# menezesandre/stackrl

Measured on AMD Instinct MI355X. Metric: env steps/sec (batched Stack-v0), higher is better.
Workload: dtype f32

## Files before the change

stackrl_amd/csrc/settle.hip:

```cpp
#include "srl_device.h"
#include "srl_kernels.h"
#include "stage.h"

#ifdef SRL_DIAG_JITTER
__device__ __forceinline__ void srl_jitter_sync() {
  unsigned t = (unsigned)__builtin_readcyclecounter() * 2654435761u + (threadIdx.x >> 6) * 40503u;
  t = __builtin_amdgcn_readfirstlane(t);
  const int n = (t >> 13) & 15;
  for (int i = 0; i < n; ++i) __builtin_amdgcn_s_sleep(16);
  __builtin_amdgcn_fence(__ATOMIC_RELEASE, "workgroup");
  __builtin_amdgcn_s_barrier();
  __builtin_amdgcn_fence(__ATOMIC_ACQUIRE, "workgroup");
  t = t * 1664525u + 1013904223u;
  const int m = (t >> 13) & 15;
  for (int i = 0; i < m; ++i) __builtin_amdgcn_s_sleep(16);
}
#define __syncthreads() srl_jitter_sync()
#endif

template <int T, int PP> struct Variant;

__device__ __forceinline__ int pair_word(int p) {
  int j = (int)((1.0f + sqrtf(1.0f + 8.0f * (float)p)) * 0.5f);
  while (j * (j - 1) / 2 > p) --j;
// ... 424 lines not shown
      if (flags & 2) {
        for (int pid = 0; pid < npair; ++pid) {
          if (L.SOP()[pid] >= 0) continue;
          int i, j; L.pair(pid, i, j);
          if (!aabb_overlap(L, i, j)) continue;
          int sl = -1;
          for (int k = 0; k < P.NS; ++k) if (L.POS()[k] < 0) { sl = k; break; }
          if (sl < 0) { misc[M_STATUS] |= SRL_ST_PAIR_OVERFLOW; atomicOr(P.flags, 4); continue; }
          L.SOP()[pid] = sl; L.POS()[sl] = pid;
          float* mp = L.MAN(sl);
          mp[0] = __int_as_float(0);
          mp[56] = __int_as_float(0);
          st3(mp + 1, ld3(L.X(i)) - ld3(L.X(j)));
        }
      }
      uint64_t* used = (uint64_t*)(L.sm + P.BLOB + P.S_USED);
      for (int b = 0; b < SRL_MAX_BODIES; ++b) used[b] = 0;
      int nc = 0;
      for (int sl = 0; sl < P.NS; ++sl) {
        int pid = L.POS()[sl];
        if (pid < 0) continue;
        int i, j; L.pair(pid, i, j);
        uint64_t u = used[i] | used[j];
        int c = __ffsll((long long)~u) - 1;
        L.COL()[sl] = c;
        used[i] |= (uint64_t)1 << c;
        used[j] |= (uint64_t)1 << c;
        if (c + 1 > nc) nc = c + 1;
      }
      misc[M_NCOL] = nc;
    }
    __syncthreads();
  }
  const int ncol = misc[M_NCOL];
  STAMP(3);
  {
    constexpr int G = VA::GJK_GROUP;
    const int gl = tid & (G - 1);
    for (int sl = tid / G; sl < P.NS; sl += T / G)
      if (L.POS()[sl] >= 0) narrowphase_slot<G>(L, sl, gl);
  }
  __syncthreads();
  STAMP(4);
  {
    GPoint gp = make_ground_point(L, tid / SRL_GMAXP, tid % SRL_GMAXP);
    if (tid / SRL_GMAXP >= nb) gp.valid = false;
    Point pp[PP];
    PSplit sp;
    if constexpr (VA::PAIR_SPLIT) {
#pragma unroll
      for (int r = 0; r < PP; ++r) pp[r].valid = slot_points(L, tid >> 2) > 0;
    } else {
#pragma unroll
    for (int r = 0; r < PP; ++r) pp[r] = make_pair_point(L, (tid + r * T) >> 2, tid & 3);
    }
    {
      bool mine = gp.valid;
#pragma unroll
      for (int r = 0; r < PP; ++r) mine |= pp[r].valid;
      if (tid >= 64 && __ballot(mine) != 0ull && (tid & 63) == 0) misc[M_SOLO] = 0;
    }
    __syncthreads();
    GBody gb;
    gb.np = 0; gb.b = 0; gb.ima = 0.0f;
    gb.pvw = L.VW(0); gb.rec = cg_rec(L, 0, 0);
#pragma unroll
    for (int i = 0; i < SRL_GMAXP; ++i) { gb.acc[i][0] = 0.0f; gb.acc[i][1] = 0.0f; gb.acc[i][2] = 0.0f; }
    constexpr bool GB = VA::GROUND_BODY, GA = VA::GROUND_AHEAD;
    if (GB) {
    if (gp.valid) cg_store(L, gp);
    if (tid < nb) {
      const float* g = L.GM(tid);
      gb.b = tid; gb.np = __float_as_int(g[0]); gb.ima = L.BC(tid)[0];
      gb.pvw = L.VW(tid); gb.rec = cg_rec(L, tid, 0);
#pragma unroll
      for (int i = 0; i < SRL_GMAXP; ++i)
        if (i < gb.np) { gb.acc[i][0] = g[SRL_GM_IN + i]; gb.acc[i][1] = g[SRL_GM_T1 + i]; gb.acc[i][2] = g[SRL_GM_T2 + i]; }
    }
    __syncthreads();
    }
    if constexpr (VA::PAIR_SPLIT) sp = make_pair_split(L, tid);
    STAMP(5);
    const bool solo = VA::SOLO && misc[M_SOLO] != 0;
    const int gslot = gp.valid ? gp.idx : -1;
    unsigned long long cm[2], cm2[2] = {0ull, 0ull};
    int pslot[PP];
    if constexpr (VA::PAIR_SPLIT) {
      const int h2 = (tid >> 1) & 1;
#pragma unroll
      for (int c = 0; c < 2; ++c) {
        cm[c] = __ballot(sp.colour == c && sp.np > 2 * h2); cm2[c] = __ballot(sp.colour == c && sp.np > 2 * h2 + 1);
      }
#pragma unroll
      for (int r = 0; r < PP; ++r) pslot[r] = -1;
    } else {
    cm[0] = __ballot(pp[0].valid && pp[0].colour == 0); cm[1] = __ballot(pp[0].valid && pp[0].colour == 1);
#pragma unroll
    for (int r = 0; r < PP; ++r) pslot[r] = pp[r].valid ? 4 * pp[r].colour + pp[r].idx : -1;
    }
    if (solo) {
      int done = 0;
      if (tid < 64) {
        bool anyp = false;
#pragma unroll
        for (int r = 0; r < PP; ++r) anyp |= pp[r].valid;
        const bool ground_only = GB && __ballot(anyp) == 0ull;
        if (ground_only) {
          v3 v = V(0.0f, 0.0f, 0.0f), w = V(0.0f, 0.0f, 0.0f);
          if (gb.np > 0) {
            vw_load(gb.pvw, v, w);
            float res = 0.0f;
            ground_body<true, false, true>(gb, P.c.warmstart, v, w, res);
          }
          for (int it = 0; it < P.c.solver_iterations; ++it) {
            done++;
            float res = 0.0f;
            if (gb.np > 0) ground_body<false, GA, true>(gb, P.c.warmstart, v, w, res);
            if (__ballot(res * res > P.c.residual_threshold) == 0ull) break;
          }
          if (gb.np > 0) vw_store(gb.pvw, v, w);
        } else {
          solver_sweep<true, T, PP, VA::SOLO>(L, gp, gb, pp, sp, ncol, gslot, pslot, 0, cm, cm2);
          for (int it = 0; it < P.c.solver_iterations; ++it) {
            done++;
            if (!solver_sweep<false, T, PP, VA::SOLO>(L, gp, gb, pp, sp, ncol, gslot, pslot, 0, cm, cm2)) break;
          }
        }
        if (tid == 0) misc[M_CNT] = done;
      }
      __syncthreads();
      gsweep += misc[M_CNT];
    } else {
      solver_sweep<true, T, PP, false>(L, gp, gb, pp, sp, ncol, gslot, pslot, 0, cm, cm2);
      for (int it = 0; it < P.c.solver_iterations; ++it) {
        gsweep++;
        if (!solver_sweep<false, T, PP, false>(L, gp, gb, pp, sp, ncol, gslot, pslot, gsweep, cm, cm2)) break;
      }
    }
#ifdef SRL_STAMPS
    if (tid == 0) {
      EnvHdr* hh = &L.P->hdr[blockIdx.x];
      bool anyp = false;
      for (int r = 0; r < PP; ++r) anyp |= pp[r].valid;
      {
        int bl[SRL_MAX_BODIES]; for (int b = 0; b < SRL_MAX_BODIES; ++b) bl[b] = 0;
        int lmax = 0, sumt = 0;
        for (int c = 0; c < ncol; ++c) {
          int mx = 0;
          for (int sl = 0; sl < P.NS; ++sl) {
            const int pid = L.POS()[sl];
            if (pid < 0 || L.COL()[sl] != c) continue;
            const int np = __float_as_int(L.MAN(sl)[0]);
            if (np <= 0) continue;
            int a, b; L.pair(pid, a, b);
            const int st = bl[a] > bl[b] ? bl[a] : bl[b];
            bl[a] = st + np; bl[b] = st + np;
            if (st + np > lmax) lmax = st + np;
            if (np > mx) mx = np;
          }
          sumt += mx;
        }
        hh->diag[4] += sumt; hh->diag[5] += lmax;
      }
      hh->diag[0] += 1; hh->diag[1] += (__ballot(anyp) == 0ull); hh->diag[2] += ncol; hh->diag[3] += solo ? misc[M_CNT] : 0;
    }
#endif
    if (!GB) {
      if (gp.valid) { float* g = L.GM(gp.a); g[SRL_GM_IN + gp.idx] = gp.in; g[SRL_GM_T1 + gp.idx] = gp.i1; g[SRL_GM_T2 + gp.idx] = gp.i2; }
    } else if (gb.np > 0) {
      float* g = L.GM(gb.b);
#pragma unroll
      for (int i = 0; i < SRL_GMAXP; ++i)
        if (i < gb.np) { g[SRL_GM_IN + i] = gb.acc[i][0]; g[SRL_GM_T1 + i] = gb.acc[i][1]; g[SRL_GM_T2 + i] = gb.acc[i][2]; }
    }
    if constexpr (VA::PAIR_SPLIT) {
      const int i0 = tid & 2;
      if (!(tid & 1) && sp.np > i0) {
        float* q = L.MAN(tid >> 2) + 4 + SRL_MP_WORDS * i0;
        q[10] = sp.s0.in; q[11] = sp.s0.i1; q[12] = sp.s0.i2;
        if (sp.np > i0 + 1) { q[SRL_MP_WORDS + 10] = sp.s1.in; q[SRL_MP_WORDS + 11] = sp.s1.i1; q[SRL_MP_WORDS + 12] = sp.s1.i2; }
      }
    } else {
#pragma unroll
    for (int r = 0; r < PP; ++r)
      if (pp[r].valid) {
        float* q = L.MAN((tid + r * T) >> 2) + 4 + SRL_MP_WORDS * pp[r].idx;
        q[10] = pp[r].in; q[11] = pp[r].i1; q[12] = pp[r].i2;
      }
    }
  }
  STAMP(6);
  const float dt = P.c.sim_time_step;
  if (tid < nb) {
    const int b = tid;
    v3 v, w;
    vw_load(L.VW(b), v, w);
    st3(L.X(b), madd(ld3(L.X(b)), v, dt));
    float* Q = L.Q(b);
    q4 q; q.x = Q[0]; q.y = Q[1]; q.z = Q[2]; q.w = Q[3];
    float hx = 0.5f * dt;
    q4 dq;
    dq.x = hx * ((w.x * q.w + w.y * q.z) - w.z * q.y);
    dq.y = hx * ((w.y * q.w + w.z * q.x) - w.x * q.z);
    dq.z = hx * ((w.z * q.w + w.x * q.y) - w.y * q.x);
    dq.w = hx * (-((w.x * q.x + w.y * q.y) + w.z * q.z));
    q.x += dq.x; q.y += dq.y; q.z += dq.z; q.w += dq.w;
    float inv = 1.0f / sqrtf((q.x * q.x + q.y * q.y) + (q.z * q.z + q.w * q.w));
    Q[0] = q.x * inv; Q[1] = q.y * inv; Q[2] = q.z * inv; Q[3] = q.w * inv;
  }
  __syncthreads();
  STAMP(7);
}

__device__ __forceinline__ bool sim_stop(const Lds& L, int nb, int tid) {
  int* misc = L.MISC();
  bool moving = false;
  if (tid < nb) {
    const float* p = L.VW(tid); const v3 v = V(p[0], p[2], p[4]);
    moving = sqrtf(dot(v, v)) > L.P->c.velocity_threshold;
// ... 376 lines not shown
```

stackrl_amd/csrc/solver.h:

```cpp
struct Row { v3 d, ca, aa, cb, ab; float rk, k; };

template <bool HAS_B>
__device__ __forceinline__ Row make_row(v3 d, v3 ra, v3 rb, float ima, const m3& Ia, float imb, const m3& Ib) {
  Row r;
  r.d = d;
  r.ca = cross(ra, d);
  r.aa = mmul(Ia, r.ca);
  r.cb = V(0.0f, 0.0f, 0.0f); r.ab = V(0.0f, 0.0f, 0.0f);
  float k = ima + dot(cross(r.aa, ra), d);
  if (HAS_B) {
    r.cb = cross(rb, d);
    r.ab = mmul(Ib, r.cb);
    k = k + (imb + dot(cross(r.ab, rb), d));
  }
  r.rk = 1.0f / k;
  r.k = k;
  return r;
}

struct PRow { f2 ka[3], kb[3], ua[3], ub[3]; float rk, k; };
struct Vel2 { f2 a[3], b[3]; };

__device__ __forceinline__ PRow pack_row(const Row& r, float ima, float imb) {
  PRow q;
  const v3 da = r.d * ima, db = r.d * (-imb);
  q.ka[0] = F2(r.d.x, r.ca.x); q.ka[1] = F2(r.d.y, r.ca.y); q.ka[2] = F2(r.d.z, r.ca.z);
  q.kb[0] = F2(r.d.x, r.cb.x); q.kb[1] = F2(r.d.y, r.cb.y); q.kb[2] = F2(r.d.z, r.cb.z);
  q.ua[0] = F2(da.x, r.aa.x); q.ua[1] = F2(da.y, r.aa.y); q.ua[2] = F2(da.z, r.aa.z);
  q.ub[0] = F2(db.x, -r.ab.x); q.ub[1] = F2(db.y, -r.ab.y); q.ub[2] = F2(db.z, -r.ab.z);
  q.rk = r.rk; q.k = r.k;
  return q;
}

__device__ __forceinline__ void prow_apply(const PRow& r, Vel2& u, float imp) {
  const f2 d2 = F2(imp, imp);
#pragma unroll
  for (int c = 0; c < 3; ++c) { u.a[c] = fma2(r.ua[c], d2, u.a[c]); u.b[c] = fma2(r.ub[c], d2, u.b[c]); }
}
__device__ __forceinline__ void prow_solve(const PRow& r, Vel2& u, float target, float& acc, float lo, float hi, float& res) {
  const f2 sa = fma2(r.ka[0], u.a[0], fma2(r.ka[1], u.a[1], r.ka[2] * u.a[2]));
  const f2 sb = fma2(r.kb[0], u.b[0], fma2(r.kb[1], u.b[1], r.kb[2] * u.b[2]));
  float ra = sa.x + sa.y;
  asm("" : "+v"(ra));
  const float vrel = ra - (sb.x + sb.y);
  float dl = fmaf(-vrel, r.rk, target * r.rk);
  const float na = __builtin_amdgcn_fmed3f(acc + dl, lo, hi);
  dl = na - acc;
  acc = na;
  res = fmaxf(res, fabsf(dl * r.k));
  prow_apply(r, u, dl);
}

__device__ __forceinline__ float contact_target(const DevParams& P, float dist) {
  float inv_dt = 1.0f / P.c.sim_time_step;
  float pen = dist + P.c.linear_slop;
  return pen > 0.0f ? -(pen * inv_dt) : -((pen * P.c.erp) * inv_dt);
}

struct Point {
  PRow n, t1, t2;
  float target, in, i1, i2, ima, imb, mu;
  int a, b;
  int colour;
  int idx;
  bool valid;
};

struct GRow { v3 ca, aa; float rk, k; };
struct GPoint {
  GRow n, t1, t2;
  float target, in, i1, i2, ima, mu;
  int a, idx;
  bool valid;
};

__device__ __forceinline__ GRow make_grow(v3 d, v3 ra, float ima, const m3& Ia) {
  GRow r;
  r.ca = cross(ra, d);
  r.aa = mmul(Ia, r.ca);
  const float k = ima + dot(cross(r.aa, ra), d);
  r.rk = 1.0f / k;
  r.k = k;
  return r;
}

template <int AXIS, int SGN>
__device__ __forceinline__ void grow_apply(v3 aa, float ima, v3& v, v3& w, float imp) {
  float& va = AXIS == 0 ? v.x : AXIS == 1 ? v.y : v.z;
  va = fmaf(SGN < 0 ? -ima : ima, imp, va);
  w = madd(w, aa, imp);
}
template <int AXIS, int SGN>
__device__ __forceinline__ void grow_solve_t(v3 ca, v3 aa, float rk, float k, float ima, v3& v, v3& w, float trk, float& acc,
                                             float lo, float hi, float& res) {
  float& va = AXIS == 0 ? v.x : AXIS == 1 ? v.y : v.z;
  const float vrel = fmaf(ca.x, w.x, fmaf(ca.y, w.y, fmaf(ca.z, w.z, SGN < 0 ? -va : va)));
  float dl = fmaf(-vrel, rk, trk);
  const float na = __builtin_amdgcn_fmed3f(acc + dl, lo, hi);
  dl = na - acc;
  acc = na;
  res = fmaxf(res, fabsf(dl * k));
  grow_apply<AXIS, SGN>(aa, ima, v, w, dl);
}
template <int AXIS, int SGN>
__device__ __forceinline__ void grow_solve(const GRow& r, float ima, v3& v, v3& w, float target, float& acc, float lo,
                                           float hi, float& res) {
  grow_solve_t<AXIS, SGN>(r.ca, r.aa, r.rk, r.k, ima, v, w, target * r.rk, acc, lo, hi, res);
}

__device__ __forceinline__ GPoint make_ground_point(const Lds& L, int b, int i) {
  const DevParams& P = *L.P;
  GPoint p;
  p.valid = false; p.a = b; p.idx = i;
  p.in = 0.0f; p.i1 = 0.0f; p.i2 = 0.0f; p.target = 0.0f; p.ima = 0.0f; p.mu = 0.0f;
  const float* g = L.GM(b);
  if (i >= __float_as_int(g[0])) return p;
  p.valid = true;
  p.ima = L.BC(b)[0];
  p.mu = P.c.friction_rock * P.c.friction_ground;
  const m3 Ia = ldm(L.IW(b));
  const int vid = __float_as_int(g[SRL_GM_VID + i]);
  const v3 pw = ld3(L.WV(b) + 3 * vid);
  const v3 ra = V(pw.x, pw.y, pw.z - P.c.collision_margin) - ld3(L.X(b));
  v3 n = V(0.0f, 0.0f, 1.0f), t1, t2;
  plane_space(n, t1, t2);
  p.n = make_grow(n, ra, p.ima, Ia);
  p.t1 = make_grow(t1, ra, p.ima, Ia);
  p.t2 = make_grow(t2, ra, p.ima, Ia);
  p.target = contact_target(P, g[SRL_GM_DIST + i]);
  p.in = g[SRL_GM_IN + i]; p.i1 = g[SRL_GM_T1 + i]; p.i2 = g[SRL_GM_T2 + i];
  return p;
}

template <bool WARM>
__device__ __forceinline__ void ground_turn(const Lds& L, GPoint& p, float& res) {
  const float ws = L.P->c.warmstart;
  v3 v, w;
  vw_load(L.VW(p.a), v, w);
  if (WARM) {
    p.in = p.in * ws; p.i1 = p.i1 * ws; p.i2 = p.i2 * ws;
    grow_apply<2, 1>(p.n.aa, p.ima, v, w, p.in);
    grow_apply<1, -1>(p.t1.aa, p.ima, v, w, p.i1);
    grow_apply<0, 1>(p.t2.aa, p.ima, v, w, p.i2);
  } else {
    grow_solve<2, 1>(p.n, p.ima, v, w, p.target, p.in, 0.0f, 1e30f, res);
    const float lim = p.mu * p.in;
    grow_solve<1, -1>(p.t1, p.ima, v, w, 0.0f, p.i1, -lim, lim, res);
    grow_solve<0, 1>(p.t2, p.ima, v, w, 0.0f, p.i2, -lim, lim, res);
  }
  vw_store(L.VW(p.a), v, w);
}

#define SRL_CG_WORDS 28
struct GBody {
  float acc[SRL_GMAXP][3];
  float ima;
  int np, b;
  float* pvw;
  const float4* rec;
};

__device__ __forceinline__ float4* cg_rec(const Lds& L, int b, int i) {
  return (float4*)L.WV(0) + (SRL_CG_WORDS / 4) * (SRL_GMAXP * b + i);
}
__device__ __forceinline__ void cg_store(const Lds& L, const GPoint& p) {
  float4* r = cg_rec(L, p.a, p.idx);
  r[0] = make_float4(p.n.ca.x, p.n.ca.y, p.n.ca.z, p.n.rk);
  r[1] = make_float4(p.n.aa.x, p.n.aa.y, p.n.aa.z, p.target * p.n.rk);
  r[2] = make_float4(p.t1.ca.x, p.t1.ca.y, p.t1.ca.z, p.t1.rk);
  r[3] = make_float4(p.t1.aa.x, p.t1.aa.y, p.t1.aa.z, p.n.k);
  r[4] = make_float4(p.t2.ca.x, p.t2.ca.y, p.t2.ca.z, p.t2.rk);
  r[5] = make_float4(p.t2.aa.x, p.t2.aa.y, p.t2.aa.z, p.t1.k);
  r[6] = make_float4(p.t2.k, p.mu, 0.0f * p.t1.rk, 0.0f * p.t2.rk);
}

struct GRec { f4 q[7]; };

template <bool WARM>
__device__ __forceinline__ void ground_point(const GRec& R, GBody& gb, int i, float ws, v3& v, v3& w, float& res) {
  const f4 q0 = R.q[0], q1 = R.q[1], q2 = R.q[2], q3 = R.q[3], q4 = R.q[4], q5 = R.q[5], q6 = R.q[6];
  if (WARM) {
    gb.acc[i][0] = gb.acc[i][0] * ws; gb.acc[i][1] = gb.acc[i][1] * ws; gb.acc[i][2] = gb.acc[i][2] * ws;
    grow_apply<2, 1>(V(q1.x, q1.y, q1.z), gb.ima, v, w, gb.acc[i][0]);
    grow_apply<1, -1>(V(q3.x, q3.y, q3.z), gb.ima, v, w, gb.acc[i][1]);
    grow_apply<0, 1>(V(q5.x, q5.y, q5.z), gb.ima, v, w, gb.acc[i][2]);
  } else {
    grow_solve_t<2, 1>(V(q0.x, q0.y, q0.z), V(q1.x, q1.y, q1.z), q0.w, q3.w, gb.ima, v, w, q1.w, gb.acc[i][0], 0.0f, 1e30f, res);
    const float lim = q6.y * gb.acc[i][0];
    grow_solve_t<1, -1>(V(q2.x, q2.y, q2.z), V(q3.x, q3.y, q3.z), q2.w, q5.w, gb.ima, v, w, q6.z, gb.acc[i][1], -lim, lim, res);
    grow_solve_t<0, 1>(V(q4.x, q4.y, q4.z), V(q5.x, q5.y, q5.z), q4.w, q6.x, gb.ima, v, w, q6.w, gb.acc[i][2], -lim, lim, res);
  }
}

__device__ __forceinline__ GRec cg_load(const float4* rec, int i) {
  GRec R;
#pragma unroll
  for (int k = 0; k < 7; ++k) { const float4 t = rec[7 * i + k]; R.q[k].x = t.x; R.q[k].y = t.y; R.q[k].z = t.z; R.q[k].w = t.w; }
  return R;
}

template <int I>
__device__ __forceinline__ void cg_request(unsigned a, GRec& R, float& tie) {
  asm volatile(
      "ds_read_b128 %0, %8 offset:%9\n\tds_read_b128 %1, %8 offset:%10\n\tds_read_b128 %2, %8 offset:%11\n\t"
      "ds_read_b128 %3, %8 offset:%12\n\tds_read_b128 %4, %8 offset:%13\n\tds_read_b128 %5, %8 offset:%14\n\t"
      "ds_read_b128 %6, %8 offset:%15"
      : "=&v"(R.q[0]), "=&v"(R.q[1]), "=&v"(R.q[2]), "=&v"(R.q[3]), "=&v"(R.q[4]), "=&v"(R.q[5]), "=&v"(R.q[6]), "+v"(tie)
      : "v"(a), "n"(112 * I), "n"(112 * I + 16), "n"(112 * I + 32), "n"(112 * I + 48), "n"(112 * I + 64), "n"(112 * I + 80),
        "n"(112 * I + 96));
}
__device__ __forceinline__ void cg_request_first(unsigned avw, unsigned a, f4& a0, f2& a1, GRec& R) {
  asm volatile(
      "ds_read_b128 %0, %9\n\tds_read_b64 %1, %9 offset:16\n\t"
      "ds_read_b128 %2, %10\n\tds_read_b128 %3, %10 offset:16\n\tds_read_b128 %4, %10 offset:32\n\t"
      "ds_read_b128 %5, %10 offset:48\n\tds_read_b128 %6, %10 offset:64\n\tds_read_b128 %7, %10 offset:80\n\t"
      "ds_read_b128 %8, %10 offset:96"
      : "=&v"(a0), "=&v"(a1), "=&v"(R.q[0]), "=&v"(R.q[1]), "=&v"(R.q[2]), "=&v"(R.q[3]), "=&v"(R.q[4]), "=&v"(R.q[5]), "=&v"(R.q[6])
      : "v"(avw), "v"(a));
}
__device__ __forceinline__ void cg_arrive_first(f4& a0, f2& a1, GRec& R) {
  asm volatile("s_waitcnt lgkmcnt(7)"
               : "+v"(a0), "+v"(a1), "+v"(R.q[0]), "+v"(R.q[1]), "+v"(R.q[2]), "+v"(R.q[3]), "+v"(R.q[4]), "+v"(R.q[5]), "+v"(R.q[6]));
}
template <int LEFT>
__device__ __forceinline__ void cg_arrive(GRec& R, float& tie) {
  asm volatile("s_waitcnt lgkmcnt(%8)"
               : "+v"(R.q[0]), "+v"(R.q[1]), "+v"(R.q[2]), "+v"(R.q[3]), "+v"(R.q[4]), "+v"(R.q[5]), "+v"(R.q[6]), "+v"(tie)
               : "n"(LEFT));
}

template <bool WARM, bool AHEAD, bool KEEP>
__device__ __forceinline__ void ground_body(GBody& gb, float ws, v3& v, v3& w, float& res) {
  static_assert(SRL_CG_WORDS == 28, "cg_request reads seven float4 per record");
  const float4* rec = gb.rec;
  static_assert(SRL_GMAXP == 4, "four nested guards below");
  if (!AHEAD) {
    if (!KEEP) vw_load(gb.pvw, v, w);
    ground_point<WARM>(cg_load(rec, 0), gb, 0, ws, v, w, res);
    if (gb.np > 1) {
      ground_point<WARM>(cg_load(rec, 1), gb, 1, ws, v, w, res);
      if (gb.np > 2) {
        ground_point<WARM>(cg_load(rec, 2), gb, 2, ws, v, w, res);
        if (gb.np > 3) ground_point<WARM>(cg_load(rec, 3), gb, 3, ws, v, w, res);
      }
    }
  } else {
    const unsigned ra = (unsigned)(size_t)rec;
    GRec r0, r1, r2, r3;
    if (!KEEP) {
      f4 a0; f2 a1;
      float none = 0.0f;
      cg_request_first((unsigned)(size_t)gb.pvw, ra, a0, a1, r0);
      cg_request<1>(ra, r1, none);
      cg_arrive_first(a0, a1, r0);
      v = V(a0.x, a0.z, a1.x); w = V(a0.y, a0.w, a1.y);
    } else {
      cg_request<0>(ra, r0, w.z);
      cg_request<1>(ra, r1, w.z);
      cg_arrive<7>(r0, w.z);
    }
    ground_point<WARM>(r0, gb, 0, ws, v, w, res);
    cg_arrive<0>(r1, w.x);
    if (gb.np > 1) {
      cg_request<2>(ra, r2, w.z);
      ground_point<WARM>(r1, gb, 1, ws, v, w, res);
      cg_arrive<0>(r2, w.x);
      if (gb.np > 2) {
        cg_request<3>(ra, r3, w.z);
        ground_point<WARM>(r2, gb, 2, ws, v, w, res);
        cg_arrive<0>(r3, w.x);
        if (gb.np > 3) ground_point<WARM>(r3, gb, 3, ws, v, w, res);
      }
    }
  }
  if (!KEEP) vw_store(gb.pvw, v, w);
}

__device__ __forceinline__ Point make_pair_point(const Lds& L, int sl, int i) {
  const DevParams& P = *L.P;
  Point p;
  p.valid = false; p.a = 0; p.b = 0; p.colour = 0; p.idx = i;
  p.in = 0.0f; p.i1 = 0.0f; p.i2 = 0.0f; p.target = 0.0f; p.ima = 0.0f; p.imb = 0.0f; p.mu = 0.0f;
  if (sl >= P.NS) return p;
  const int pid = L.POS()[sl];
  if (pid < 0) return p;
  const float* mp = L.MAN(sl);
  if (i >= __float_as_int(mp[0])) return p;
  p.valid = true;
  L.pair(pid, p.a, p.b);
  p.colour = L.COL()[sl];
  p.ima = L.BC(p.a)[0]; p.imb = L.BC(p.b)[0];
  p.mu = P.c.friction_rock * P.c.friction_rock;
  const float* q = mp + 4 + SRL_MP_WORDS * i;
  const m3 Ra = ldm(L.R(p.a)), Rb = ldm(L.R(p.b));
  const m3 Ia = ldm(L.IW(p.a)), Ib = ldm(L.IW(p.b));
  const v3 ra = mmul(Ra, ld3(q));
  const v3 rb = mmul(Rb, ld3(q + 3));
  v3 n = ld3(q + 6), t1, t2;
  plane_space(n, t1, t2);
  p.n = pack_row(make_row<true>(n, ra, rb, p.ima, Ia, p.imb, Ib), p.ima, p.imb);
  p.t1 = pack_row(make_row<true>(t1, ra, rb, p.ima, Ia, p.imb, Ib), p.ima, p.imb);
  p.t2 = pack_row(make_row<true>(t2, ra, rb, p.ima, Ia, p.imb, Ib), p.ima, p.imb);
  p.target = contact_target(P, q[9]);
  p.in = q[10]; p.i1 = q[11]; p.i2 = q[12];
  return p;
}

template <bool WARM>
__device__ __forceinline__ void point_turn(const Lds& L, Point& p, float& res) {
  const float ws = L.P->c.warmstart;
  Vel2 u;
  float* const pa = L.VW(p.a);
  float* const pb = L.VW(p.b);
  vw_load(pa, u.a);
  vw_load(pb, u.b);
  if (WARM) {
    p.in = p.in * ws; p.i1 = p.i1 * ws; p.i2 = p.i2 * ws;
    prow_apply(p.n, u, p.in);
    prow_apply(p.t1, u, p.i1);
    prow_apply(p.t2, u, p.i2);
  } else {
    prow_solve(p.n, u, p.target, p.in, 0.0f, 1e30f, res);
    const float lim = p.mu * p.in;
    prow_solve(p.t1, u, 0.0f, p.i1, -lim, lim, res);
    prow_solve(p.t2, u, 0.0f, p.i2, -lim, lim, res);
  }
  vw_store(pa, u.a);
  vw_store(pb, u.b);
}

struct HRow { f2 k[3], u[3]; float rk, kk; };
struct HSet { HRow n, t1, t2; float trk, in, i1, i2; };
struct PSplit {
  HSet s0, s1;
  float* pvw;
  int np;
  int colour;
  float mu;
};

__device__ __forceinline__ float quad_partner(float x) {
  return __int_as_float(__builtin_amdgcn_update_dpp(0, __float_as_int(x), 0xB1, 0xf, 0xf, true));
}

__device__ __forceinline__ HRow make_hrow(v3 d, v3 r, float im, const m3& I, bool side) {
  HRow h;
  const v3 c = cross(r, d);
  const v3 a = mmul(I, c);
  const float part = im + dot(cross(a, r), d);
  const float k = part + quad_partner(part);
  const v3 dm = d * (side ? -im : im);
  h.k[0] = side ? F2(-d.x, -c.x) : F2(d.x, c.x); h.k[1] = side ? F2(-d.y, -c.y) : F2(d.y, c.y); h.k[2] = side ? F2(-d.z, -c.z) : F2(d.z, c.z);
  h.u[0] = F2(dm.x, side ? -a.x : a.x); h.u[1] = F2(dm.y, side ? -a.y : a.y); h.u[2] = F2(dm.z, side ? -a.z : a.z);
  h.rk = 1.0f / k; h.kk = k;
  return h;
}

__device__ __forceinline__ HSet make_hset(const Lds& L, const float* mp, int i, int np, int body, bool side) {
  const DevParams& P = *L.P;
  HSet s;
  s.trk = 0.0f; s.in = 0.0f; s.i1 = 0.0f; s.i2 = 0.0f;
  if (i >= np) {
    HRow z;
    z.k[0] = z.k[1] = z.k[2] = z.u[0] = z.u[1] = z.u[2] = F2(0.0f, 0.0f); z.rk = 0.0f; z.kk = 0.0f;
    s.n = z; s.t1 = z; s.t2 = z;
    return s;
  }
  const float im = L.BC(body)[0];
  const float* q = mp + 4 + SRL_MP_WORDS * i;
  const v3 r = mmul(ldm(L.R(body)), ld3(q + (side ? 3 : 0)));
  const m3 I = ldm(L.IW(body));
  v3 n = ld3(q + 6), t1, t2;
  plane_space(n, t1, t2);
  s.n = make_hrow(n, r, im, I, side);
  s.t1 = make_hrow(t1, r, im, I, side);
  s.t2 = make_hrow(t2, r, im, I, side);
  s.trk = contact_target(P, q[9]) * s.n.rk;
  s.in = q[10]; s.i1 = q[11]; s.i2 = q[12];
  return s;
}

__device__ __forceinline__ int slot_points(const Lds& L, int sl) {
  if (sl >= L.P->NS || L.POS()[sl] < 0) return 0;
  return __float_as_int(L.MAN(sl)[0]);
}

__device__ __forceinline__ PSplit make_pair_split(const Lds& L, int tid) {
  const DevParams& P = *L.P;
  const int sl = tid >> 2, h = (tid >> 1) & 1;
  const bool side = tid & 1;
  PSplit p;
  p.np = 0; p.colour = 0; p.pvw = L.VW(0);
  p.mu = P.c.friction_rock * P.c.friction_rock;
  int body = 0;
  const float* mp = L.MAN(0);
  if (sl < P.NS) {
    const int pid = L.POS()[sl];
    if (pid >= 0) {
      int a, b; L.pair(pid, a, b);
      body = side ? b : a;
      mp = L.MAN(sl);
      p.np = __float_as_int(mp[0]);
      p.colour = L.COL()[sl];
      p.pvw = L.VW(body);
    }
  }
  p.s0 = make_hset(L, mp, 2 * h, p.np, body, side);
  p.s1 = make_hset(L, mp, 2 * h + 1, p.np, body, side);
  return p;
}

__device__ __forceinline__ void hrow_apply(const HRow& r, f2 (&u)[3], f2 d2) {
#pragma unroll
  for (int c = 0; c < 3; ++c) u[c] = fma2(r.u[c], d2, u[c]);
}
__device__ __forceinline__ void hrow_solve(const HRow& r, f2 (&u)[3], float trk, float& acc, float lo, float hi, float& res) {
  const f2 s = fma2(r.k[0], u[0], fma2(r.k[1], u[1], r.k[2] * u[2]));
  float own = s.x + s.y;
  asm("" : "+v"(own));
  const float vrel = own + quad_partner(own);
  float dl = fmaf(-vrel, r.rk, trk);
  const float na = __builtin_amdgcn_fmed3f(acc + dl, lo, hi);
  dl = na - acc;
  acc = na;
  res = fmaxf(res, fabsf(dl * r.kk));
  hrow_apply(r, u, F2(dl, dl));
}

__device__ __forceinline__ float zero_times(float rk) {
  float t;
  asm volatile("v_mul_f32 %0, 0, %1" : "=v"(t) : "v"(rk));
  return t;
}

template <bool WARM>
__device__ __forceinline__ void hset_turn(HSet& s, f2 (&u)[3], float mu, float ws, float& res) {
  if (WARM) {
    s.in = s.in * ws; s.i1 = s.i1 * ws; s.i2 = s.i2 * ws;
    const f2 dn = F2(s.in, s.in), d1 = F2(s.i1, s.i1), d2 = F2(s.i2, s.i2);
    hrow_apply(s.n, u, dn);
    hrow_apply(s.t1, u, d1);
    hrow_apply(s.t2, u, d2);
  } else {
    hrow_solve(s.n, u, s.trk, s.in, 0.0f, 1e30f, res);
    const float lim = mu * s.in;
    hrow_solve(s.t1, u, zero_times(s.t1.rk), s.i1, -lim, lim, res);
    hrow_solve(s.t2, u, zero_times(s.t2.rk), s.i2, -lim, lim, res);
  }
}

template <bool WARM>
__device__ __forceinline__ void pair_phase(PSplit& p, float ws, unsigned long long m1, unsigned long long m2, float& res) {
  constexpr unsigned long long LO = 0x3333333333333333ull;
#pragma unroll
  for (int h = 0; h < 2; ++h) {
    const unsigned long long t1 = m1 & (LO << (2 * h)), t2 = m2 & (LO << (2 * h));
    if (t1 == 0) return;
    if (__builtin_amdgcn_inverse_ballot_w64(t1)) {
      f2 u[3];
      vw_load(p.pvw, u);
      hset_turn<WARM>(p.s0, u, p.mu, ws, res);
      if (t2 != 0) {
        if (__builtin_amdgcn_inverse_ballot_w64(t2)) hset_turn<WARM>(p.s1, u, p.mu, ws, res);
      }
      vw_store(p.pvw, u);
    }
    __builtin_amdgcn_wave_barrier();
    if (t2 == 0) return;
  }
}

template <bool WARM, int T, int PP, bool SOLO>
__device__ __forceinline__ bool solver_sweep(const Lds& L, GPoint& gp, GBody& gb, Point (&pp)[PP], PSplit& sp, int ncol, int gslot,
                                             const int (&pslot)[PP], int gsweep, const unsigned long long (&cm)[2],
                                             const unsigned long long (&cm2)[2]) {
  typedef Variant<T, PP> VA;
  static_assert(!SOLO || VA::SOLO, "a solo sweep in a variant that has none");
  float res = 0.0f;
  constexpr unsigned long long T0 = 0x1111111111111111ull;
  if (!VA::GROUND_BODY) {
    const unsigned long long gm = __ballot(gslot >= 0);
#pragma unroll
    for (int i = 0; i < SRL_GMAXP; ++i) {
      const unsigned long long t = gm & (T0 << i);
      if (t == 0) break;
      if (__builtin_amdgcn_inverse_ballot_w64(t)) ground_turn<WARM>(L, gp, res);
      __builtin_amdgcn_wave_barrier();
    }
  } else {
    v3 v, w;
    if (gb.np > 0) ground_body<WARM, !WARM && VA::GROUND_AHEAD, false>(gb, L.P->c.warmstart, v, w, res);
    __builtin_amdgcn_wave_barrier();
  }
  int c0 = 0;
  if (SOLO) {
#pragma unroll
    for (int c = 0; c < 2; ++c) {
      if (c >= ncol) break;
      if constexpr (VA::PAIR_SPLIT) {
        pair_phase<WARM>(sp, L.P->c.warmstart, cm[c], cm2[c], res);
      } else {
#pragma unroll
      for (int i = 0; i < 4; ++i) {
        const unsigned long long t = cm[c] & (T0 << i);
        if (t == 0) break;
        if (__builtin_amdgcn_inverse_ballot_w64(t)) point_turn<WARM>(L, pp[0], res);
        __builtin_amdgcn_wave_barrier();
      }
      }
    }
    c0 = 2;
  }
#pragma unroll 1
  for (int c = c0; c < ncol; ++c) {
    if (!SOLO) __syncthreads();
    if constexpr (VA::PAIR_SPLIT) {
      const int h2 = (threadIdx.x >> 1) & 1;
      const bool mine = sp.colour == c;
      pair_phase<WARM>(sp, L.P->c.warmstart, __ballot(mine && sp.np > 2 * h2), __ballot(mine && sp.np > 2 * h2 + 1), res);
    } else {
    unsigned long long mc[PP];
#pragma unroll
    for (int r = 0; r < PP; ++r) mc[r] = __ballot((pslot[r] >> 2) == c);
#pragma unroll
    for (int i = 0; i < 4; ++i) {
      unsigned long long any = 0;
#pragma unroll
      for (int r = 0; r < PP; ++r) any |= mc[r] & (T0 << i);
      if (any == 0) break;
#pragma unroll
      for (int r = 0; r < PP; ++r)
        if (__builtin_amdgcn_inverse_ballot_w64(mc[r] & (T0 << i))) point_turn<WARM>(L, pp[r], res);
      __builtin_amdgcn_wave_barrier();
    }
    }
  }
  if (SOLO) return WARM ? true : __ballot(res * res > L.P->c.residual_threshold) != 0ull;
  int* word = L.MISC() + M_RES0 + (gsweep & 1);
  if (!WARM) {
    if (__ballot(res * res > L.P->c.residual_threshold) != 0ull && (threadIdx.x & 63) == 0) *word = gsweep;
  }
  __syncthreads();
  return WARM ? true : *word == gsweep;
}
```

Measured before the change: 112,700.

## Compact ground contact records and specialise friction rows

Ground contact rows exploit the fixed normal/tangent axes so only the non-zero cross-product components are stored and used, shrinking each LDS record from seven float4 to five and cutting the FMAs in the ground solve. Friction mu is hoisted to a wave-uniform scalar passed into the sweeps instead of being stored per record. Friction rows in pair and split solves use a template specialisation with a pre-negated rk, dropping the zero-target multiply and the inline asm helper. This reduces LDS traffic and VALU work in the inner solver loop but relies on the plane_space basis having the assumed zero pattern.

```diff
diff --git a/stackrl_amd/csrc/settle.hip b/stackrl_amd/csrc/settle.hip
--- a/stackrl_amd/csrc/settle.hip
+++ b/stackrl_amd/csrc/settle.hip
@@ -530,6 +530,7 @@
     if constexpr (VA::PAIR_SPLIT) sp = make_pair_split(L, tid);
     STAMP(5);
     const bool solo = VA::SOLO && misc[M_SOLO] != 0;
+    const float gmu = __int_as_float(__builtin_amdgcn_readfirstlane(__float_as_int(ground_mu(P.c))));
     const int gslot = gp.valid ? gp.idx : -1;
     unsigned long long cm[2], cm2[2] = {0ull, 0ull};
     int pslot[PP];
@@ -558,20 +559,20 @@
           if (gb.np > 0) {
             vw_load(gb.pvw, v, w);
             float res = 0.0f;
-            ground_body<true, false, true>(gb, P.c.warmstart, v, w, res);
+            ground_body<true, false, true>(gb, P.c.warmstart, gmu, v, w, res);
           }
           for (int it = 0; it < P.c.solver_iterations; ++it) {
             done++;
             float res = 0.0f;
-            if (gb.np > 0) ground_body<false, GA, true>(gb, P.c.warmstart, v, w, res);
+            if (gb.np > 0) ground_body<false, GA, true>(gb, P.c.warmstart, gmu, v, w, res);
             if (__ballot(res * res > P.c.residual_threshold) == 0ull) break;
           }
           if (gb.np > 0) vw_store(gb.pvw, v, w);
         } else {
-          solver_sweep<true, T, PP, VA::SOLO>(L, gp, gb, pp, sp, ncol, gslot, pslot, 0, cm, cm2);
+          solver_sweep<true, T, PP, VA::SOLO>(L, gp, gb, pp, sp, ncol, gslot, pslot, 0, cm, cm2, gmu);
           for (int it = 0; it < P.c.solver_iterations; ++it) {
             done++;
-            if (!solver_sweep<false, T, PP, VA::SOLO>(L, gp, gb, pp, sp, ncol, gslot, pslot, 0, cm, cm2)) break;
+            if (!solver_sweep<false, T, PP, VA::SOLO>(L, gp, gb, pp, sp, ncol, gslot, pslot, 0, cm, cm2, gmu)) break;
           }
         }
         if (tid == 0) misc[M_CNT] = done;
@@ -579,10 +580,10 @@
       __syncthreads();
       gsweep += misc[M_CNT];
     } else {
-      solver_sweep<true, T, PP, false>(L, gp, gb, pp, sp, ncol, gslot, pslot, 0, cm, cm2);
+      solver_sweep<true, T, PP, false>(L, gp, gb, pp, sp, ncol, gslot, pslot, 0, cm, cm2, gmu);
       for (int it = 0; it < P.c.solver_iterations; ++it) {
         gsweep++;
-        if (!solver_sweep<false, T, PP, false>(L, gp, gb, pp, sp, ncol, gslot, pslot, gsweep, cm, cm2)) break;
+        if (!solver_sweep<false, T, PP, false>(L, gp, gb, pp, sp, ncol, gslot, pslot, gsweep, cm, cm2, gmu)) break;
       }
     }
 #ifdef SRL_STAMPS
diff --git a/stackrl_amd/csrc/solver.h b/stackrl_amd/csrc/solver.h
--- a/stackrl_amd/csrc/solver.h
+++ b/stackrl_amd/csrc/solver.h
@@ -37,13 +37,14 @@
 #pragma unroll
   for (int c = 0; c < 3; ++c) { u.a[c] = fma2(r.ua[c], d2, u.a[c]); u.b[c] = fma2(r.ub[c], d2, u.b[c]); }
 }
+template <bool FRICTION>
 __device__ __forceinline__ void prow_solve(const PRow& r, Vel2& u, float target, float& acc, float lo, float hi, float& res) {
   const f2 sa = fma2(r.ka[0], u.a[0], fma2(r.ka[1], u.a[1], r.ka[2] * u.a[2]));
   const f2 sb = fma2(r.kb[0], u.b[0], fma2(r.kb[1], u.b[1], r.kb[2] * u.b[2]));
   float ra = sa.x + sa.y;
   asm("" : "+v"(ra));
   const float vrel = ra - (sb.x + sb.y);
-  float dl = fmaf(-vrel, r.rk, target * r.rk);
+  float dl = FRICTION ? vrel * r.rk : fmaf(-vrel, r.rk, target * r.rk);
   const float na = __builtin_amdgcn_fmed3f(acc + dl, lo, hi);
   dl = na - acc;
   acc = na;
@@ -66,18 +67,21 @@
   bool valid;
 };
 
-struct GRow { v3 ca, aa; float rk, k; };
+struct GRow { v3 aa; float rk, k; };
 struct GPoint {
   GRow n, t1, t2;
-  float target, in, i1, i2, ima, mu;
+  float c[4];
+  float target, in, i1, i2, ima;
   int a, idx;
   bool valid;
 };
 
-__device__ __forceinline__ GRow make_grow(v3 d, v3 ra, float ima, const m3& Ia) {
+__device__ __forceinline__ float ground_mu(const srl_config& c) { return c.friction_rock * c.friction_ground; }
+
+__device__ __forceinline__ GRow make_grow(v3 d, v3 ra, float ima, const m3& Ia, v3& ca) {
   GRow r;
-  r.ca = cross(ra, d);
-  r.aa = mmul(Ia, r.ca);
+  ca = cross(ra, d);
+  r.aa = mmul(Ia, ca);
   const float k = ima + dot(cross(r.aa, ra), d);
   r.rk = 1.0f / k;
   r.k = k;
@@ -91,11 +95,12 @@
   w = madd(w, aa, imp);
 }
 template <int AXIS, int SGN>
-__device__ __forceinline__ void grow_solve_t(v3 ca, v3 aa, float rk, float k, float ima, v3& v, v3& w, float trk, float& acc,
-                                             float lo, float hi, float& res) {
+__device__ __forceinline__ void grow_solve_t(float c0, float c1, v3 aa, float rk, float k, float ima, v3& v, v3& w, float trk,
+                                             float& acc, float lo, float hi, float& res) {
   float& va = AXIS == 0 ? v.x : AXIS == 1 ? v.y : v.z;
-  const float vrel = fmaf(ca.x, w.x, fmaf(ca.y, w.y, fmaf(ca.z, w.z, SGN < 0 ? -va : va)));
-  float dl = fmaf(-vrel, rk, trk);
+  const float w0 = AXIS == 0 ? w.y : w.x, w1 = AXIS == 2 ? w.y : w.z;
+  const float vrel = fmaf(c0, w0, fmaf(c1, w1, SGN < 0 ? -va : va));
+  float dl = AXIS != 2 ? vrel * rk : fmaf(-vrel, rk, trk);
   const float na = __builtin_amdgcn_fmed3f(acc + dl, lo, hi);
   dl = na - acc;
   acc = na;
@@ -103,37 +108,39 @@
   grow_apply<AXIS, SGN>(aa, ima, v, w, dl);
 }
 template <int AXIS, int SGN>
-__device__ __forceinline__ void grow_solve(const GRow& r, float ima, v3& v, v3& w, float target, float& acc, float lo,
-                                           float hi, float& res) {
-  grow_solve_t<AXIS, SGN>(r.ca, r.aa, r.rk, r.k, ima, v, w, target * r.rk, acc, lo, hi, res);
+__device__ __forceinline__ void grow_solve(float c0, float c1, const GRow& r, float ima, v3& v, v3& w, float target, float& acc,
+                                           float lo, float hi, float& res) {
+  grow_solve_t<AXIS, SGN>(c0, c1, r.aa, r.rk, r.k, ima, v, w, target * r.rk, acc, lo, hi, res);
 }
 
 __device__ __forceinline__ GPoint make_ground_point(const Lds& L, int b, int i) {
   const DevParams& P = *L.P;
   GPoint p;
   p.valid = false; p.a = b; p.idx = i;
-  p.in = 0.0f; p.i1 = 0.0f; p.i2 = 0.0f; p.target = 0.0f; p.ima = 0.0f; p.mu = 0.0f;
+  p.in = 0.0f; p.i1 = 0.0f; p.i2 = 0.0f; p.target = 0.0f; p.ima = 0.0f;
   const float* g = L.GM(b);
   if (i >= __float_as_int(g[0])) return p;
   p.valid = true;
   p.ima = L.BC(b)[0];
-  p.mu = P.c.friction_rock * P.c.friction_ground;
   const m3 Ia = ldm(L.IW(b));
   const int vid = __float_as_int(g[SRL_GM_VID + i]);
   const v3 pw = ld3(L.WV(b) + 3 * vid);
   const v3 ra = V(pw.x, pw.y, pw.z - P.c.collision_margin) - ld3(L.X(b));
   v3 n = V(0.0f, 0.0f, 1.0f), t1, t2;
   plane_space(n, t1, t2);
-  p.n = make_grow(n, ra, p.ima, Ia);
-  p.t1 = make_grow(t1, ra, p.ima, Ia);
-  p.t2 = make_grow(t2, ra, p.ima, Ia);
+  v3 cn, c1, c2;
+  p.n = make_grow(n, ra, p.ima, Ia, cn);
+  p.t1 = make_grow(t1, ra, p.ima, Ia, c1);
+  p.t2 = make_grow(t2, ra, p.ima, Ia, c2);
+  p.c[0] = cn.x; p.c[1] = cn.y; p.c[2] = c1.x; p.c[3] = c2.z;
+  p.t1.rk = -p.t1.rk; p.t2.rk = -p.t2.rk;
   p.target = contact_target(P, g[SRL_GM_DIST + i]);
   p.in = g[SRL_GM_IN + i]; p.i1 = g[SRL_GM_T1 + i]; p.i2 = g[SRL_GM_T2 + i];
   return p;
 }
 
 template <bool WARM>
-__device__ __forceinline__ void ground_turn(const Lds& L, GPoint& p, float& res) {
+__device__ __forceinline__ void ground_turn(const Lds& L, GPoint& p, float mu, float& res) {
   const float ws = L.P->c.warmstart;
   v3 v, w;
   vw_load(L.VW(p.a), v, w);
@@ -143,15 +150,15 @@
     grow_apply<1, -1>(p.t1.aa, p.ima, v, w, p.i1);
     grow_apply<0, 1>(p.t2.aa, p.ima, v, w, p.i2);
   } else {
-    grow_solve<2, 1>(p.n, p.ima, v, w, p.target, p.in, 0.0f, 1e30f, res);
-    const float lim = p.mu * p.in;
-    grow_solve<1, -1>(p.t1, p.ima, v, w, 0.0f, p.i1, -lim, lim, res);
-    grow_solve<0, 1>(p.t2, p.ima, v, w, 0.0f, p.i2, -lim, lim, res);
+    grow_solve<2, 1>(p.c[0], p.c[1], p.n, p.ima, v, w, p.target, p.in, 0.0f, 1e30f, res);
+    const float lim = mu * p.in;
+    grow_solve<1, -1>(p.c[2], p.c[1], p.t1, p.ima, v, w, 0.0f, p.i1, -lim, lim, res);
+    grow_solve<0, 1>(p.c[2], p.c[3], p.t2, p.ima, v, w, 0.0f, p.i2, -lim, lim, res);
   }
   vw_store(L.VW(p.a), v, w);
 }
 
-#define SRL_CG_WORDS 28
+#define SRL_CG_WORDS 20
 struct GBody {
   float acc[SRL_GMAXP][3];
   float ima;
@@ -165,83 +172,78 @@
 }
 __device__ __forceinline__ void cg_store(const Lds& L, const GPoint& p) {
   float4* r = cg_rec(L, p.a, p.idx);
-  r[0] = make_float4(p.n.ca.x, p.n.ca.y, p.n.ca.z, p.n.rk);
-  r[1] = make_float4(p.n.aa.x, p.n.aa.y, p.n.aa.z, p.target * p.n.rk);
-  r[2] = make_float4(p.t1.ca.x, p.t1.ca.y, p.t1.ca.z, p.t1.rk);
-  r[3] = make_float4(p.t1.aa.x, p.t1.aa.y, p.t1.aa.z, p.n.k);
-  r[4] = make_float4(p.t2.ca.x, p.t2.ca.y, p.t2.ca.z, p.t2.rk);
-  r[5] = make_float4(p.t2.aa.x, p.t2.aa.y, p.t2.aa.z, p.t1.k);
-  r[6] = make_float4(p.t2.k, p.mu, 0.0f * p.t1.rk, 0.0f * p.t2.rk);
-}
-
-struct GRec { f4 q[7]; };
+  r[0] = make_float4(p.c[0], p.c[1], p.n.rk, p.target * p.n.rk);
+  r[1] = make_float4(p.n.aa.x, p.n.aa.y, p.n.aa.z, p.n.k);
+  r[2] = make_float4(p.c[2], p.c[3], p.t1.rk, p.t2.rk);
+  r[3] = make_float4(p.t1.aa.x, p.t1.aa.y, p.t1.aa.z, p.t1.k);
+  r[4] = make_float4(p.t2.aa.x, p.t2.aa.y, p.t2.aa.z, p.t2.k);
+}
+
+struct GRec { f4 q[5]; };
 
 template <bool WARM>
-__device__ __forceinline__ void ground_point(const GRec& R, GBody& gb, int i, float ws, v3& v, v3& w, float& res) {
-  const f4 q0 = R.q[0], q1 = R.q[1], q2 = R.q[2], q3 = R.q[3], q4 = R.q[4], q5 = R.q[5], q6 = R.q[6];
+__device__ __forceinline__ void ground_point(const GRec& R, GBody& gb, int i, float ws, float mu, v3& v, v3& w, float& res) {
+  const f4 q0 = R.q[0], q1 = R.q[1], q2 = R.q[2], q3 = R.q[3], q4 = R.q[4];
   if (WARM) {
     gb.acc[i][0] = gb.acc[i][0] * ws; gb.acc[i][1] = gb.acc[i][1] * ws; gb.acc[i][2] = gb.acc[i][2] * ws;
     grow_apply<2, 1>(V(q1.x, q1.y, q1.z), gb.ima, v, w, gb.acc[i][0]);
     grow_apply<1, -1>(V(q3.x, q3.y, q3.z), gb.ima, v, w, gb.acc[i][1]);
-    grow_apply<0, 1>(V(q5.x, q5.y, q5.z), gb.ima, v, w, gb.acc[i][2]);
+    grow_apply<0, 1>(V(q4.x, q4.y, q4.z), gb.ima, v, w, gb.acc[i][2]);
   } else {
-    grow_solve_t<2, 1>(V(q0.x, q0.y, q0.z), V(q1.x, q1.y, q1.z), q0.w, q3.w, gb.ima, v, w, q1.w, gb.acc[i][0], 0.0f, 1e30f, res);
-    const float lim = q6.y * gb.acc[i][0];
-    grow_solve_t<1, -1>(V(q2.x, q2.y, q2.z), V(q3.x, q3.y, q3.z), q2.w, q5.w, gb.ima, v, w, q6.z, gb.acc[i][1], -lim, lim, res);
-    grow_solve_t<0, 1>(V(q4.x, q4.y, q4.z), V(q5.x, q5.y, q5.z), q4.w, q6.x, gb.ima, v, w, q6.w, gb.acc[i][2], -lim, lim, res);
+    grow_solve_t<2, 1>(q0.x, q0.y, V(q1.x, q1.y, q1.z), q0.z, q1.w, gb.ima, v, w, q0.w, gb.acc[i][0], 0.0f, 1e30f, res);
+    const float lim = mu * gb.acc[i][0];
+    grow_solve_t<1, -1>(q2.x, q0.y, V(q3.x, q3.y, q3.z), q2.z, q3.w, gb.ima, v, w, 0.0f, gb.acc[i][1], -lim, lim, res);
+    grow_solve_t<0, 1>(q2.x, q2.y, V(q4.x, q4.y, q4.z), q2.w, q4.w, gb.ima, v, w, 0.0f, gb.acc[i][2], -lim, lim, res);
   }
 }
 
 __device__ __forceinline__ GRec cg_load(const float4* rec, int i) {
   GRec R;
 #pragma unroll
-  for (int k = 0; k < 7; ++k) { const float4 t = rec[7 * i + k]; R.q[k].x = t.x; R.q[k].y = t.y; R.q[k].z = t.z; R.q[k].w = t.w; }
+  for (int k = 0; k < 5; ++k) { const float4 t = rec[5 * i + k]; R.q[k].x = t.x; R.q[k].y = t.y; R.q[k].z = t.z; R.q[k].w = t.w; }
   return R;
 }
 
 template <int I>
 __device__ __forceinline__ void cg_request(unsigned a, GRec& R, float& tie) {
   asm volatile(
-      "ds_read_b128 %0, %8 offset:%9\n\tds_read_b128 %1, %8 offset:%10\n\tds_read_b128 %2, %8 offset:%11\n\t"
-      "ds_read_b128 %3, %8 offset:%12\n\tds_read_b128 %4, %8 offset:%13\n\tds_read_b128 %5, %8 offset:%14\n\t"
-      "ds_read_b128 %6, %8 offset:%15"
-      : "=&v"(R.q[0]), "=&v"(R.q[1]), "=&v"(R.q[2]), "=&v"(R.q[3]), "=&v"(R.q[4]), "=&v"(R.q[5]), "=&v"(R.q[6]), "+v"(tie)
-      : "v"(a), "n"(112 * I), "n"(112 * I + 16), "n"(112 * I + 32), "n"(112 * I + 48), "n"(112 * I + 64), "n"(112 * I + 80),
-        "n"(112 * I + 96));
+      "ds_read_b128 %0, %6 offset:%7\n\tds_read_b128 %1, %6 offset:%8\n\tds_read_b128 %2, %6 offset:%9\n\t"
+      "ds_read_b128 %3, %6 offset:%10\n\tds_read_b128 %4, %6 offset:%11"
+      : "=&v"(R.q[0]), "=&v"(R.q[1]), "=&v"(R.q[2]), "=&v"(R.q[3]), "=&v"(R.q[4]), "+v"(tie)
+      : "v"(a), "n"(80 * I), "n"(80 * I + 16), "n"(80 * I + 32), "n"(80 * I + 48), "n"(80 * I + 64));
 }
 __device__ __forceinline__ void cg_request_first(unsigned avw, unsigned a, f4& a0, f2& a1, GRec& R) {
   asm volatile(
-      "ds_read_b128 %0, %9\n\tds_read_b64 %1, %9 offset:16\n\t"
-      "ds_read_b128 %2, %10\n\tds_read_b128 %3, %10 offset:16\n\tds_read_b128 %4, %10 offset:32\n\t"
-      "ds_read_b128 %5, %10 offset:48\n\tds_read_b128 %6, %10 offset:64\n\tds_read_b128 %7, %10 offset:80\n\t"
-      "ds_read_b128 %8, %10 offset:96"
-      : "=&v"(a0), "=&v"(a1), "=&v"(R.q[0]), "=&v"(R.q[1]), "=&v"(R.q[2]), "=&v"(R.q[3]), "=&v"(R.q[4]), "=&v"(R.q[5]), "=&v"(R.q[6])
+      "ds_read_b128 %0, %7\n\tds_read_b64 %1, %7 offset:16\n\t"
+      "ds_read_b128 %2, %8\n\tds_read_b128 %3, %8 offset:16\n\tds_read_b128 %4, %8 offset:32\n\t"
+      "ds_read_b128 %5, %8 offset:48\n\tds_read_b128 %6, %8 offset:64"
+      : "=&v"(a0), "=&v"(a1), "=&v"(R.q[0]), "=&v"(R.q[1]), "=&v"(R.q[2]), "=&v"(R.q[3]), "=&v"(R.q[4])
       : "v"(avw), "v"(a));
 }
 __device__ __forceinline__ void cg_arrive_first(f4& a0, f2& a1, GRec& R) {
-  asm volatile("s_waitcnt lgkmcnt(7)"
-               : "+v"(a0), "+v"(a1), "+v"(R.q[0]), "+v"(R.q[1]), "+v"(R.q[2]), "+v"(R.q[3]), "+v"(R.q[4]), "+v"(R.q[5]), "+v"(R.q[6]));
+  asm volatile("s_waitcnt lgkmcnt(5)"
+               : "+v"(a0), "+v"(a1), "+v"(R.q[0]), "+v"(R.q[1]), "+v"(R.q[2]), "+v"(R.q[3]), "+v"(R.q[4]));
 }
 template <int LEFT>
 __device__ __forceinline__ void cg_arrive(GRec& R, float& tie) {
-  asm volatile("s_waitcnt lgkmcnt(%8)"
-               : "+v"(R.q[0]), "+v"(R.q[1]), "+v"(R.q[2]), "+v"(R.q[3]), "+v"(R.q[4]), "+v"(R.q[5]), "+v"(R.q[6]), "+v"(tie)
+  asm volatile("s_waitcnt lgkmcnt(%6)"
+               : "+v"(R.q[0]), "+v"(R.q[1]), "+v"(R.q[2]), "+v"(R.q[3]), "+v"(R.q[4]), "+v"(tie)
                : "n"(LEFT));
 }
 
 template <bool WARM, bool AHEAD, bool KEEP>
-__device__ __forceinline__ void ground_body(GBody& gb, float ws, v3& v, v3& w, float& res) {
-  static_assert(SRL_CG_WORDS == 28, "cg_request reads seven float4 per record");
+__device__ __forceinline__ void ground_body(GBody& gb, float ws, float mu, v3& v, v3& w, float& res) {
+  static_assert(SRL_CG_WORDS == 20, "cg_request reads five float4 per record");
   const float4* rec = gb.rec;
   static_assert(SRL_GMAXP == 4, "four nested guards below");
   if (!AHEAD) {
     if (!KEEP) vw_load(gb.pvw, v, w);
-    ground_point<WARM>(cg_load(rec, 0), gb, 0, ws, v, w, res);
+    ground_point<WARM>(cg_load(rec, 0), gb, 0, ws, mu, v, w, res);
     if (gb.np > 1) {
-      ground_point<WARM>(cg_load(rec, 1), gb, 1, ws, v, w, res);
+      ground_point<WARM>(cg_load(rec, 1), gb, 1, ws, mu, v, w, res);
       if (gb.np > 2) {
-        ground_point<WARM>(cg_load(rec, 2), gb, 2, ws, v, w, res);
-        if (gb.np > 3) ground_point<WARM>(cg_load(rec, 3), gb, 3, ws, v, w, res);
+        ground_point<WARM>(cg_load(rec, 2), gb, 2, ws, mu, v, w, res);
+        if (gb.np > 3) ground_point<WARM>(cg_load(rec, 3), gb, 3, ws, mu, v, w, res);
       }
     }
   } else {
@@ -257,19 +259,19 @@
     } else {
       cg_request<0>(ra, r0, w.z);
       cg_request<1>(ra, r1, w.z);
-      cg_arrive<7>(r0, w.z);
-    }
-    ground_point<WARM>(r0, gb, 0, ws, v, w, res);
+      cg_arrive<5>(r0, w.z);
+    }
+    ground_point<WARM>(r0, gb, 0, ws, mu, v, w, res);
     cg_arrive<0>(r1, w.x);
     if (gb.np > 1) {
       cg_request<2>(ra, r2, w.z);
-      ground_point<WARM>(r1, gb, 1, ws, v, w, res);
+      ground_point<WARM>(r1, gb, 1, ws, mu, v, w, res);
       cg_arrive<0>(r2, w.x);
       if (gb.np > 2) {
         cg_request<3>(ra, r3, w.z);
-        ground_point<WARM>(r2, gb, 2, ws, v, w, res);
+        ground_point<WARM>(r2, gb, 2, ws, mu, v, w, res);
         cg_arrive<0>(r3, w.x);
-        if (gb.np > 3) ground_point<WARM>(r3, gb, 3, ws, v, w, res);
+        if (gb.np > 3) ground_point<WARM>(r3, gb, 3, ws, mu, v, w, res);
       }
     }
   }
@@ -301,6 +303,7 @@
   p.n = pack_row(make_row<true>(n, ra, rb, p.ima, Ia, p.imb, Ib), p.ima, p.imb);
   p.t1 = pack_row(make_row<true>(t1, ra, rb, p.ima, Ia, p.imb, Ib), p.ima, p.imb);
   p.t2 = pack_row(make_row<true>(t2, ra, rb, p.ima, Ia, p.imb, Ib), p.ima, p.imb);
+  p.t1.rk = -p.t1.rk; p.t2.rk = -p.t2.rk;
   p.target = contact_target(P, q[9]);
   p.in = q[10]; p.i1 = q[11]; p.i2 = q[12];
   return p;
@@ -320,10 +323,10 @@
     prow_apply(p.t1, u, p.i1);
     prow_apply(p.t2, u, p.i2);
   } else {
-    prow_solve(p.n, u, p.target, p.in, 0.0f, 1e30f, res);
+    prow_solve<false>(p.n, u, p.target, p.in, 0.0f, 1e30f, res);
     const float lim = p.mu * p.in;
-    prow_solve(p.t1, u, 0.0f, p.i1, -lim, lim, res);
-    prow_solve(p.t2, u, 0.0f, p.i2, -lim, lim, res);
+    prow_solve<true>(p.t1, u, 0.0f, p.i1, -lim, lim, res);
+    prow_solve<true>(p.t2, u, 0.0f, p.i2, -lim, lim, res);
   }
   vw_store(pa, u.a);
   vw_store(pb, u.b);
@@ -375,6 +378,7 @@
   s.n = make_hrow(n, r, im, I, side);
   s.t1 = make_hrow(t1, r, im, I, side);
   s.t2 = make_hrow(t2, r, im, I, side);
+  s.t1.rk = -s.t1.rk; s.t2.rk = -s.t2.rk;
   s.trk = contact_target(P, q[9]) * s.n.rk;
   s.in = q[10]; s.i1 = q[11]; s.i2 = q[12];
   return s;
@@ -414,23 +418,18 @@
 #pragma unroll
   for (int c = 0; c < 3; ++c) u[c] = fma2(r.u[c], d2, u[c]);
 }
+template <bool FRICTION>
 __device__ __forceinline__ void hrow_solve(const HRow& r, f2 (&u)[3], float trk, float& acc, float lo, float hi, float& res) {
   const f2 s = fma2(r.k[0], u[0], fma2(r.k[1], u[1], r.k[2] * u[2]));
   float own = s.x + s.y;
   asm("" : "+v"(own));
   const float vrel = own + quad_partner(own);
-  float dl = fmaf(-vrel, r.rk, trk);
+  float dl = FRICTION ? vrel * r.rk : fmaf(-vrel, r.rk, trk);
   const float na = __builtin_amdgcn_fmed3f(acc + dl, lo, hi);
   dl = na - acc;
   acc = na;
   res = fmaxf(res, fabsf(dl * r.kk));
   hrow_apply(r, u, F2(dl, dl));
-}
-
-__device__ __forceinline__ float zero_times(float rk) {
-  float t;
-  asm volatile("v_mul_f32 %0, 0, %1" : "=v"(t) : "v"(rk));
-  return t;
 }
 
 template <bool WARM>
@@ -442,10 +441,10 @@
     hrow_apply(s.t1, u, d1);
     hrow_apply(s.t2, u, d2);
   } else {
-    hrow_solve(s.n, u, s.trk, s.in, 0.0f, 1e30f, res);
+    hrow_solve<false>(s.n, u, s.trk, s.in, 0.0f, 1e30f, res);
     const float lim = mu * s.in;
-    hrow_solve(s.t1, u, zero_times(s.t1.rk), s.i1, -lim, lim, res);
-    hrow_solve(s.t2, u, zero_times(s.t2.rk), s.i2, -lim, lim, res);
+    hrow_solve<true>(s.t1, u, 0.0f, s.i1, -lim, lim, res);
+    hrow_solve<true>(s.t2, u, 0.0f, s.i2, -lim, lim, res);
   }
 }
 
@@ -473,7 +472,7 @@
 template <bool WARM, int T, int PP, bool SOLO>
 __device__ __forceinline__ bool solver_sweep(const Lds& L, GPoint& gp, GBody& gb, Point (&pp)[PP], PSplit& sp, int ncol, int gslot,
                                              const int (&pslot)[PP], int gsweep, const unsigned long long (&cm)[2],
-                                             const unsigned long long (&cm2)[2]) {
+                                             const unsigned long long (&cm2)[2], float gmu) {
   typedef Variant<T, PP> VA;
   static_assert(!SOLO || VA::SOLO, "a solo sweep in a variant that has none");
   float res = 0.0f;
@@ -484,12 +483,12 @@
     for (int i = 0; i < SRL_GMAXP; ++i) {
       const unsigned long long t = gm & (T0 << i);
       if (t == 0) break;
-      if (__builtin_amdgcn_inverse_ballot_w64(t)) ground_turn<WARM>(L, gp, res);
+      if (__builtin_amdgcn_inverse_ballot_w64(t)) ground_turn<WARM>(L, gp, gmu, res);
       __builtin_amdgcn_wave_barrier();
     }
   } else {
     v3 v, w;
-    if (gb.np > 0) ground_body<WARM, !WARM && VA::GROUND_AHEAD, false>(gb, L.P->c.warmstart, v, w, res);
+    if (gb.np > 0) ground_body<WARM, !WARM && VA::GROUND_AHEAD, false>(gb, L.P->c.warmstart, gmu, v, w, res);
     __builtin_amdgcn_wave_barrier();
   }
   int c0 = 0;
```

Measured after the change: 115,700, median of 6. 1.03x the previous value.
